# liruihui/Dis-PU

Measured on AMD Instinct MI355X. Metric: upsampled points/sec (256->1024, 4x), higher is better.
Workload: dtype f32; 1 GPU; BASELINE configs[1]: 32 patches x 256 points per GPU, generator forward 256->1024 (4x), fp32; patches_per_gpu=32, global_patches=32, weights=xavier-uniform seed 1234, zero bias, parallelism=patch-sharded x1

## Files before the change

dis-pu_amd/csrc/edge.hip:

```cpp
#include "common.h"
#include "knn_select.h"


namespace dispu {

typedef float f32x16 __attribute__((ext_vector_type(16)));

template <int CTRL>
__device__ __forceinline__ float edge_dpp(float identity, float v) {
    return __int_as_float(__builtin_amdgcn_update_dpp(__float_as_int(identity), __float_as_int(v), CTRL, 0xF, 0xF, false));
}
__device__ __forceinline__ float edge_row16_max(float v) {
    v = fmaxf(v, edge_dpp<0x121>(v, v));
    v = fmaxf(v, edge_dpp<0x122>(v, v));
    v = fmaxf(v, edge_dpp<0x124>(v, v));
    v = fmaxf(v, edge_dpp<0x128>(v, v));
    return v;
}

__device__ __forceinline__ void edge_fill_frag(float* frag, const float* __restrict__ W, int K, int tid, int nthreads) {
    const int nf4 = K * 24 / 4;
    for (int e = tid; e < nf4; e += nthreads) {
        const float4 v = *reinterpret_cast<const float4*>(W + e * 4);
        const int k = (e * 4) / 24, ch0 = (e * 4) - k * 24;
        const float vv[4] = {v.x, v.y, v.z, v.w};
#pragma unroll
        for (int u = 0; u < 4; ++u) {
            const int ch = ch0 + u, r = ch >> 1, hp = ch & 1;
            const int i = (r & 3) | (hp << 2) | ((r >> 2) << 3);
            frag[(k >> 1) * 64 + (k & 1) * 32 + i] = vv[u];
        }
    }
    for (int e = tid; e < K * 8; e += nthreads) {
        const int sh = e >> 3;
        frag[sh * 32 + 24 + (e & 7)] = 0.f;
    }
}

__device__ __forceinline__ void edge_scatter_f4(float* frag, int e, const float4 v) {
    const int k = (e * 4) / 24, ch0 = (e * 4) - k * 24;
    const float vv[4] = {v.x, v.y, v.z, v.w};
#pragma unroll
    for (int u = 0; u < 4; ++u) {
        const int ch = ch0 + u, r = ch >> 1, hp = ch & 1;
        const int i = (r & 3) | (hp << 2) | ((r >> 2) << 3);
        frag[(k >> 1) * 64 + (k & 1) * 32 + i] = vv[u];
    }
}

constexpr int EK_NP = 64 * 4 + 4;
constexpr int EK_SCRATCH = 128 + 4;
constexpr int EK_KLD = 20;
// ... 68 lines not shown
                        const float x = xr[k];
                        const float4 w = *reinterpret_cast<const float4*>(Wl + k * 24 + q * 4);
                        acc.x = __builtin_fmaf(x, w.x, acc.x); acc.y = __builtin_fmaf(x, w.y, acc.y);
                        acc.z = __builtin_fmaf(x, w.z, acc.z); acc.w = __builtin_fmaf(x, w.w, acc.w);
                    }
                    const float4 b = *reinterpret_cast<const float4*>(bl + q * 4);
                    acc.x = acc.x + b.x; acc.y = acc.y + b.y; acc.z = acc.z + b.z; acc.w = acc.w + b.w;
                    cv[u] = acc;
                    const int pl = p - (g_lo * 2 - cloud0);
                    if (e < ctotal && pl >= 0 && pl < (g_hi - g_lo) * 2)
                        *reinterpret_cast<float4*>(Lout + (size_t)(cloud0 + p) * ldl + q * 4) = acc;
                }
            }
        } else {
#pragma unroll
            for (int u = 0; u < CB; ++u) {
                const int e = min((int)threadIdx.x + u * NT, ctotal - 1);
                const int p = e / (C / 4), q = e - p * (C / 4);
                cv[u] = *reinterpret_cast<const float4*>(F + (size_t)(cloud0 + p) * ldf + q * 4);
            }
        }
#pragma unroll
        for (int u = 0; u < WB; ++u) {
            const int e = (int)threadIdx.x + u * NT;
            if (e < N0) edge_scatter_f4(f0, e, wv[u]);
            else if (e < N0 + N1) edge_scatter_f4(f1, e - N0, wv[u]);
            else if (e < N0 + N1 + N2) edge_scatter_f4(f2, e - N0 - N1, wv[u]);
        }
        for (int e = threadIdx.x; e < (K0 + K1 + K2) * 8; e += NT)
            frag[(e >> 3) * 32 + 24 + (e & 7)] = 0.f;
#pragma unroll
        for (int u = 0; u < CB; ++u) {
            const int e = (int)threadIdx.x + u * NT;
            const int p = e / (C / 4), q = e - p * (C / 4);
            if (e < ctotal) *reinterpret_cast<float4*>(fl + p * FLD + q * 4) = cv[u];
        }
        if (!layer0)
            for (int e = threadIdx.x + CB * NT; e < ctotal; e += NT) {
                const int p = e / (C / 4), q = e - p * (C / 4);
                *reinterpret_cast<float4*>(fl + p * FLD + q * 4) = *reinterpret_cast<const float4*>(F + (size_t)(cloud0 + p) * ldf + q * 4);
            }
    }
    __syncthreads();
#ifdef EDGE_STAMPS
    const unsigned long long e_ka = __builtin_readcyclecounter();
    unsigned long long e_kb = e_ka, e_kc = e_ka;
#endif
    const int lane = threadIdx.x & 63, wave = threadIdx.x >> 6;
    const int row = lane & 31, h = lane >> 5;
    float* pre = fl + n_per_cloud * FLD;
    float* norms = pre + per_wg * 2 * 24;
    uint32_t* dmat = reinterpret_cast<uint32_t*>(norms + ((n_per_cloud + 3) & ~3));
    uint64_t* kscr = reinterpret_cast<uint64_t*>(dmat + EK_MAXQ * EK_NP);
    int* nbr = reinterpret_cast<int*>(kscr + NWAVE * EK_SCRATCH);
    const int n = n_per_cloud, p_base = g_lo * 2 - cloud0, ngl = g_hi - g_lo, nq = ngl * 2;
    typedef float ek_f32x4 __attribute__((ext_vector_type(4)));
    ek_f32x4 d00 = {0.f, 0.f, 0.f, 0.f}, d01 = d00, d10 = d00, d11 = d00;
    const int i16 = lane & 15, q4 = lane >> 4;
    const int ntile = (n + 15) >> 4;
    if constexpr (KNN) {
        for (int p = threadIdx.x; p < n; p += 64 * NWAVE) {
            const float* fr = fl + p * FLD;
            float r = 0.f;
#pragma unroll
            for (int c4 = 0; c4 < C / 4; ++c4) {
                const float4 v = *reinterpret_cast<const float4*>(fr + c4 * 4);
                r = __builtin_fmaf(v.x, v.x, r); r = __builtin_fmaf(v.y, v.y, r);
                r = __builtin_fmaf(v.z, v.z, r); r = __builtin_fmaf(v.w, v.w, r);
            }
            norms[p] = r;
        }
        if (wave < ntile) {
            const float* q0row = fl + min(p_base + i16, n - 1) * FLD + q4;
            const float* q1row = fl + min(p_base + 16 + i16, n - 1) * FLD + q4;
            const float* c0p = fl + min(wave * 16 + i16, n - 1) * FLD + q4;
            const float* c1p = fl + min((wave + NWAVE) * 16 + i16, n - 1) * FLD + q4;
#pragma unroll
            for (int c4 = 0; c4 < C / 4; ++c4) {
                const float a0 = q0row[c4 * 4], a1 = q1row[c4 * 4], b0v = c0p[c4 * 4], b1v = c1p[c4 * 4];
                d00 = __builtin_amdgcn_mfma_f32_16x16x4f32(a0, b0v, d00, 0, 0, 0);
                d01 = __builtin_amdgcn_mfma_f32_16x16x4f32(a0, b1v, d01, 0, 0, 0);
                d10 = __builtin_amdgcn_mfma_f32_16x16x4f32(a1, b0v, d10, 0, 0, 0);
                d11 = __builtin_amdgcn_mfma_f32_16x16x4f32(a1, b1v, d11, 0, 0, 0);
            }
        }
    }
    if constexpr (PRE) {
        const int npts_wg = nq;
        const int tw = KNN ? NWAVE - 1 - wave : wave;
        for (int t = tw; t * 32 < npts_wg; t += NWAVE) {
            const int pl = min(t * 32 + row, npts_wg - 1);
            const float* fr = fl + (p_base + pl) * FLD;
            f32x16 acc;
#pragma unroll
            for (int r = 0; r < 16; ++r) acc[r] = 0.f;
#pragma unroll
            for (int sq = 0; sq < C / 4; ++sq) {
                const float4 a = *reinterpret_cast<const float4*>(fr + sq * 4);
                acc = __builtin_amdgcn_mfma_f32_32x32x2f32(f0[(2 * sq) * 64 + lane], h ? a.y : a.x, acc, 0, 0, 0);
                acc = __builtin_amdgcn_mfma_f32_32x32x2f32(f0[(2 * sq + 1) * 64 + lane], h ? a.w : a.z, acc, 0, 0, 0);
            }
            if (t * 32 + row < npts_wg) {
                float* pp = pre + ((t * 32 + row) * 2 + h) * 12;
#pragma unroll
                for (int q = 0; q < 3; ++q)
                    *reinterpret_cast<float4*>(pp + q * 4) = make_float4(acc[4 * q], acc[4 * q + 1], acc[4 * q + 2], acc[4 * q + 3]);
            }
        }
        __syncthreads();
    }
#ifdef EDGE_STAMPS
    e_kb = __builtin_readcyclecounter();
#endif
    if constexpr (KNN) {
        if (wave < ntile) {
            const int cand0 = wave * 16 + i16, cand1 = cand0 + NWAVE * 16;
            const float rp0 = norms[min(cand0, n - 1)], rp1 = norms[min(cand1, n - 1)];
#pragma unroll
            for (int r = 0; r < 4; ++r) {
                const float rq0 = norms[min(p_base + 4 * q4 + r, n - 1)], rq1 = norms[min(p_base + 16 + 4 * q4 + r, n - 1)];
                uint32_t* m0 = dmat + (4 * q4 + r) * EK_NP;
                uint32_t* m1 = m0 + 16 * EK_NP;
                if (cand0 < n) {
                    m0[cand0] = f32_to_ordered(((rq0 - 2.0f * d00[r]) + rp0) + 0.0f);
                    if (nq > 16) m1[cand0] = f32_to_ordered(((rq1 - 2.0f * d10[r]) + rp0) + 0.0f);
                }
                if (cand1 < n) {
                    m0[cand1] = f32_to_ordered(((rq0 - 2.0f * d01[r]) + rp1) + 0.0f);
                    if (nq > 16) m1[cand1] = f32_to_ordered(((rq1 - 2.0f * d11[r]) + rp1) + 0.0f);
                }
            }
        }
        __syncthreads();
#ifdef EDGE_STAMPS
        e_kc = __builtin_readcyclecounter();
#endif
    }
    auto knn_select = [&](int gl) {
        if constexpr (KNN) {
            const int qa = 2 * gl, qb = qa + 1;
            uint32_t oda[4], odb[4];
            int cp[4];
#pragma unroll
            for (int r = 0; r < 4; ++r) {
                const int p = lane + 64 * r;
                cp[r] = p;
                oda[r] = (p < n) ? dmat[qa * EK_NP + p] : 0xFFFFFFFFu;
                odb[r] = (p < n) ? dmat[qb * EK_NP + p] : 0xFFFFFFFFu;
            }
            uint64_t* buf = kscr + (size_t)wave * EK_SCRATCH;
            int* outa = nbr + qa * EK_KLD;
            int* outb = nbr + qb * EK_KLD;
            const auto w2f = [](uint32_t w) { return ordered_to_f32(w); };
            const bool done_a = prefilter_rank<4, true>(oda, cp, buf, lane, ksel, 0xFFFFFFFEu, outa, nullptr, w2f);
            const bool done_b = prefilter_rank<4, true>(odb, cp, buf, lane, ksel, 0xFFFFFFFEu, outb, nullptr, w2f);
            if (!(done_a && done_b)) {
                uint64_t ka[4], kb[4];
#pragma unroll
                for (int r = 0; r < 4; ++r) {
                    ka[r] = (cp[r] < n) ? (((uint64_t)oda[r] << 32) | (uint32_t)cp[r]) : KEY_MAX;
                    kb[r] = (cp[r] < n) ? (((uint64_t)odb[r] << 32) | (uint32_t)cp[r]) : KEY_MAX;
                }
                sort_keys<4>(ka);
                sort_keys<4>(kb);
                uint64_t resa, resb;
                select_k2<4>(ka, kb, lane, ksel, resa, resb);
                if (lane < ksel) {
                    if (!done_a) outa[lane] = (int)(uint32_t)resa;
                    if (!done_b) outb[lane] = (int)(uint32_t)resb;
                }
            }
            if (idx_out != nullptr && lane < ksel) {
                int* o = idx_out + (size_t)(cloud0 + p_base + qa) * ksel;
                o[lane] = outa[lane];
                o[ksel + lane] = outb[lane];
            }
        }
    };
    if constexpr (KNN) {
        for (int gl = wave; gl < ngl; gl += NWAVE) knn_select(gl);
    }
#ifdef EDGE_STAMPS
    const unsigned long long e_k1 = __builtin_readcyclecounter();
#endif

    const int ngroups = LDSF ? g_hi : (npoints + 1) / 2;
    const int s_nb = row & 15;
    float4 ra[LDSF ? 1 : C / 4], rb[LDSF ? 1 : C / 4];
    int jl_next = 0;
    auto fetch = [&](int grp) {
        int p = grp * 2 + (row >> 4);
        if (p >= npoints) p = npoints - 1;
        if constexpr (KNN) {
            jl_next = nbr[(p - g_lo * 2) * EK_KLD + ioff + s_nb];
        } else if constexpr (LDSF) {
            jl_next = idx[(size_t)p * ldi + ioff + s_nb];
        } else {
            const int j = (p / n_per_cloud) * n_per_cloud + idx[(size_t)p * ldi + ioff + s_nb];
#pragma unroll
            for (int q = 0; q < C / 4; ++q) {
                ra[q] = *reinterpret_cast<const float4*>(F + (size_t)p * ldf + q * 4);
                rb[q] = *reinterpret_cast<const float4*>(F + (size_t)j * ldf + q * 4);
            }
        }
    };
    const int grp0 = gfirst + wave, gstride = gstep0;
    if (grp0 < ngroups) fetch(grp0);
    constexpr int SKIP = PRE ? H : 0;
    constexpr int WD = 12, STOT = S0 + S1 + S2 - SKIP;
    static_assert(STOT % WD == 0, "fragment ring depth must divide the step count");
    const float* fragG = frag + SKIP * 64;
    float wq[WD];
#pragma unroll
    for (int i = 0; i < WD; ++i) wq[i] = fragG[i * 64 + lane];
#ifdef EDGE_STAMPS
    unsigned long long e_conv = 0, e_l0 = 0, e_l1 = 0, e_l2 = 0, e_epi = 0, e_n = 0;
#define ED_T(v) __builtin_amdgcn_sched_barrier(0); const unsigned long long v = __builtin_readcyclecounter(); __builtin_amdgcn_sched_barrier(0)
#else
#define ED_T(v)
#endif
    float tail_bias = 0.f;
    if constexpr (KNN) {
        if (Wp != nullptr) tail_bias = bp[min(wave >> 1, 2) * 16 + i16];
    }
    for (int grp = grp0; grp < ngroups; grp += gstride) {
        ED_T(t0);
        float fp[H], df[H];
        const float* fp_ = fl + (grp * 2 + (row >> 4) - cloud0) * FLD;
        const float* fj_ = fl + jl_next * FLD;
#pragma unroll
        for (int q = 0; q < C / 4; ++q) {
            const float4 a = LDSF ? *reinterpret_cast<const float4*>(fp_ + q * 4) : ra[q];
            const float4 b = LDSF ? *reinterpret_cast<const float4*>(fj_ + q * 4) : rb[q];
            const float a0 = h ? a.y : a.x, a1 = h ? a.w : a.z;
            const float b0v = h ? b.y : b.x, b1v = h ? b.w : b.z;
            fp[2 * q] = a0; fp[2 * q + 1] = a1;
            df[2 * q] = b0v - a0; df[2 * q + 1] = b1v - a1;
        }
        if (grp + gstride < ngroups) fetch(grp + gstride);
        f32x16 l0, l1, l2;
#pragma unroll
        for (int r = 0; r < 16; ++r) { l0[r] = 0.f; l1[r] = 0.f; l2[r] = 0.f; }
        if constexpr (PRE) {
            const float* pp = pre + (((grp - g_lo) * 2 + (row >> 4)) * 2 + h) * 12;
#pragma unroll
            for (int q = 0; q < 3; ++q) {
                const float4 v = *reinterpret_cast<const float4*>(pp + q * 4);
                l0[4 * q] = v.x; l0[4 * q + 1] = v.y; l0[4 * q + 2] = v.z; l0[4 * q + 3] = v.w;
            }
        }
        auto step = [&](int sg, float bv, f32x16& acc) {
            const float w = wq[sg % WD];
            wq[sg % WD] = fragG[((sg + WD) % STOT) * 64 + lane];
            acc = __builtin_amdgcn_mfma_f32_32x32x2f32(w, bv, acc, 0, 0, 0);
        };
        ED_T(t1);
#pragma unroll
        for (int s = SKIP; s < S0; ++s) {
            const float bv = (s < H) ? fp[s < H ? s : 0] : df[s < H ? 0 : s - H];
            step(s - SKIP, bv, l0);
        }
#pragma unroll
        for (int r = 0; r < 12; ++r) l0[r] = fmaxf(l0[r] + b0[2 * r + h], 0.f);
        ED_T(t2);
#pragma unroll
        for (int s = 0; s < S1; ++s) {
            const float bv = (s < 12) ? l0[s < 12 ? s : 0] : fp[s < 12 ? 0 : s - 12];
            step(S0 - SKIP + s, bv, l1);
        }
#pragma unroll
        for (int r = 0; r < 12; ++r) l1[r] = fmaxf(l1[r] + b1[2 * r + h], 0.f);
        ED_T(t3);
#pragma unroll
        for (int s = 0; s < S2; ++s) {
            const float bv = (s < 12) ? l1[s < 12 ? s : 0] : ((s < 24) ? l0[(s >= 12 && s < 24) ? s - 12 : 0] : fp[s >= 24 ? s - 24 : 0]);
            step(S0 + S1 - SKIP + s, bv, l2);
        }
// ... 1 lines not shown
        constexpr int OW = 3 * G + C;
        float* stg = stage + (KNN ? (grp - g_lo) : wave) * (2 * OWS);
        float* sp = stg + (row >> 4) * OWS;
        float k2 = 0.f, k1 = 0.f, k0 = 0.f;
#pragma unroll
        for (int r = 0; r < 12; ++r) {
            float m2 = l2[r] + b2[2 * r + h], m1 = l1[r], m0 = l0[r];
            asm("s_nop 1\n\t"
                "v_max_f32_dpp %0, %0, %0 row_ror:1 row_mask:0xf bank_mask:0xf\n\t"
                "v_max_f32_dpp %1, %1, %1 row_ror:1 row_mask:0xf bank_mask:0xf\n\t"
                "v_max_f32_dpp %2, %2, %2 row_ror:1 row_mask:0xf bank_mask:0xf\n\t"
                "v_max_f32_dpp %0, %0, %0 row_ror:2 row_mask:0xf bank_mask:0xf\n\t"
                "v_max_f32_dpp %1, %1, %1 row_ror:2 row_mask:0xf bank_mask:0xf\n\t"
                "v_max_f32_dpp %2, %2, %2 row_ror:2 row_mask:0xf bank_mask:0xf\n\t"
                "v_max_f32_dpp %0, %0, %0 row_ror:4 row_mask:0xf bank_mask:0xf\n\t"
                "v_max_f32_dpp %1, %1, %1 row_ror:4 row_mask:0xf bank_mask:0xf\n\t"
                "v_max_f32_dpp %2, %2, %2 row_ror:4 row_mask:0xf bank_mask:0xf\n\t"
                "v_max_f32_dpp %0, %0, %0 row_ror:8 row_mask:0xf bank_mask:0xf\n\t"
                "v_max_f32_dpp %1, %1, %1 row_ror:8 row_mask:0xf bank_mask:0xf\n\t"
                "v_max_f32_dpp %2, %2, %2 row_ror:8 row_mask:0xf bank_mask:0xf"
                : "+v"(m2), "+v"(m1), "+v"(m0));
            k2 = (s_nb == r) ? m2 : k2; k1 = (s_nb == r) ? m1 : k1; k0 = (s_nb == r) ? m0 : k0;
        }
        if (s_nb < 12) { sp[2 * s_nb + h] = k2; sp[G + 2 * s_nb + h] = k1; sp[2 * G + 2 * s_nb + h] = k0; }
        {
            float fa = 0.f, fb = 0.f;
#pragma unroll
            for (int t = 0; t < H; ++t) {
                if (t < 16) fa = (s_nb == t) ? fp[t] : fa;
                else fb = (s_nb == t - 16) ? fp[t] : fb;
            }
            if (s_nb < (H < 16 ? H : 16)) sp[3 * G + 2 * s_nb + h] = fa;
            if (H > 16 && s_nb < H - 16) sp[3 * G + 2 * (s_nb + 16) + h] = fb;
        }
        const int p_first = grp * 2;
        if (vec_store) {
            if (lane < 2 * (OW / 4)) {
                const int pt = lane / (OW / 4), q4 = lane - pt * (OW / 4);
                if (p_first + pt < npoints)
                    *reinterpret_cast<float4*>(Y + (size_t)(p_first + pt) * ldy + q4 * 4) = *reinterpret_cast<const float4*>(stg + pt * OWS + q4 * 4);
            }
        } else {
            for (int e = lane; e < 2 * OW; e += 64) {
                const int pt = e / OW, q = e - pt * OW;
                if (p_first + pt < npoints) Y[(size_t)(p_first + pt) * ldy + q] = stg[pt * OWS + q];
            }
        }
#ifdef EDGE_STAMPS
        { ED_T(t5); e_conv += t1 - t0; e_l0 += t2 - t1; e_l1 += t3 - t2; e_l2 += t4 - t3; e_epi += t5 - t4; ++e_n; }
#endif
    }
#ifdef EDGE_STAMPS
    const unsigned long long e_p0 = __builtin_readcyclecounter();
    unsigned long long e_p1 = e_p0, e_p2 = e_p0, e_p3 = e_p0;
#endif
    if constexpr (KNN) {
        if (Wp != nullptr) {
            constexpr int OW = 3 * G + C, NT = 64 * NWAVE;
            const int K = OW + k_old, xld = k_old + 4;
            float* wl = fl;
            float* xl = frag;
            __syncthreads();
#ifdef EDGE_STAMPS
            e_p1 = __builtin_readcyclecounter();
#endif
            const int wtot = K * 12, xq = k_old >> 2, xtot = nq * xq;
            constexpr int TB_W = 9, TB_X = 4;
            float4 wv[TB_W], xv[TB_X];
#pragma unroll
            for (int u = 0; u < TB_W; ++u) wv[u] = *reinterpret_cast<const float4*>(Wp + (size_t)min((int)threadIdx.x + u * NT, wtot - 1) * 4);
#pragma unroll
            for (int u = 0; u < TB_X; ++u) {
                const int e = min((int)threadIdx.x + u * NT, max(xtot - 1, 0));
                const int pl = xq ? e / xq : 0, c4 = e - pl * xq;
                xv[u] = xtot ? *reinterpret_cast<const float4*>(Y + (size_t)(g_lo * 2 + pl) * ldy + OW + c4 * 4) : make_float4(0.f, 0.f, 0.f, 0.f);
            }
#pragma unroll
            for (int u = 0; u < TB_W; ++u) {
                const int e = (int)threadIdx.x + u * NT;
                if (e < wtot) *reinterpret_cast<float4*>(wl + e * 4) = wv[u];
            }
#pragma unroll
            for (int u = 0; u < TB_X; ++u) {
                const int e = (int)threadIdx.x + u * NT;
                const int pl = xq ? e / xq : 0, c4 = e - pl * xq;
                if (e < xtot) *reinterpret_cast<float4*>(xl + pl * xld + c4 * 4) = xv[u];
            }
            for (int e = threadIdx.x + TB_W * NT; e < wtot; e += NT)
                *reinterpret_cast<float4*>(wl + e * 4) = *reinterpret_cast<const float4*>(Wp + (size_t)e * 4);
            for (int e = threadIdx.x + TB_X * NT; e < xtot; e += NT) {
                const int pl = e / xq, c4 = e - pl * xq;
                *reinterpret_cast<float4*>(xl + pl * xld + c4 * 4) = *reinterpret_cast<const float4*>(Y + (size_t)(g_lo * 2 + pl) * ldy + OW + c4 * 4);
            }
            __syncthreads();
#ifdef EDGE_STAMPS
            e_p2 = __builtin_readcyclecounter();
#endif
            const int pt = wave & 1, ct = wave >> 1;
            if (ct < 3 && pt * 16 < nq) {
                const int pl = min(pt * 16 + i16, nq - 1);
                const float* xn = stage + pl * OWS + q4;
                const float* xo = xl + pl * xld + q4;
                const float* wp = wl + q4 * 48 + ct * 16 + i16;
                ek_f32x4 acc = {0.f, 0.f, 0.f, 0.f};
                const int nround = K / 24;
                float av[6], bv[6], an[6], bn[6];
                auto rd_load = [&](int rd, float (&a)[6], float (&b)[6]) {
                    rd = min(rd, nround - 1);
                    const float* xa = (rd < OW / 24) ? xn + rd * 24 : xo + (rd - OW / 24) * 24;
                    const float* wb = wp + rd * 24 * 48;
#pragma unroll
                    for (int u = 0; u < 6; ++u) { a[u] = xa[u * 4]; b[u] = wb[u * 4 * 48]; }
                };
                rd_load(0, av, bv);
                for (int rd = 0; rd < nround; rd += 2) {
                    rd_load(rd + 1, an, bn);
#pragma unroll
                    for (int u = 0; u < 6; ++u) acc = __builtin_amdgcn_mfma_f32_16x16x4f32(av[u], bv[u], acc, 0, 0, 0);
                    if (rd + 1 < nround) {
                        rd_load(rd + 2, av, bv);
#pragma unroll
                        for (int u = 0; u < 6; ++u) acc = __builtin_amdgcn_mfma_f32_16x16x4f32(an[u], bn[u], acc, 0, 0, 0);
                    }
                }
#ifdef EDGE_STAMPS
                __builtin_amdgcn_sched_barrier(0); e_p3 = __builtin_readcyclecounter(); __builtin_amdgcn_sched_barrier(0);
#endif
                const float bb = tail_bias;
#pragma unroll
                for (int r = 0; r < 4; ++r) {
                    const int pr = pt * 16 + 4 * q4 + r;
                    if (pr < nq) Pout[(size_t)(g_lo * 2 + pr) * ldp + ct * 16 + i16] = fmaxf(acc[r] + bb, 0.f);
                }
            }
        }
    }
#ifdef EDGE_STAMPS
    if (blockIdx.x == 3 && blockIdx.y == 0 && lane == 0) {
        unsigned long long* st = reinterpret_cast<unsigned long long*>(Y + (size_t)npoints * ldy) + wave * 16;
        st[11] = e_p1 - e_p0; st[12] = e_p2 - e_p1; st[13] = __builtin_readcyclecounter() - e_p2; st[14] = e_p3 - e_p2;
        st[0] = e_conv; st[1] = e_l0; st[2] = e_l1; st[3] = e_l2; st[4] = e_epi; st[5] = e_n; st[6] = e_ka - e_k0; st[7] = e_kb - e_ka;
        st[8] = e_kc - e_kb; st[9] = e_k1 - e_kc; st[10] = __builtin_readcyclecounter() - e_k0;
    }
#endif
}

}

using namespace dispu;

DISPU_EXPORT int dispu_edge_dense_conv(int npoints, int n_per_cloud, int C, const float* F, long ldf, const int* idx, int ldi,
                                       int ioff, const float* W0, const float* b0, const float* W1, const float* b1,
                                       const float* W2, const float* b2, float* Y, long ldy, void* stream) {
    if (npoints < 0 || n_per_cloud <= 0 || !(C == 24 || C == 48) || (ldf & 3) || (((uintptr_t)F) & 15)) return (int)hipErrorInvalidValue;
    if (npoints == 0) return 0;
    hipStream_t s = (hipStream_t)stream;
    const size_t frag_bytes = (size_t)((C == 24 ? 84 : 132) * 64 + 16 * (72 + C)) * sizeof(float);
    const size_t feat_bytes = (size_t)n_per_cloud * (C + 4) * sizeof(float);
    if (npoints % n_per_cloud == 0 && n_per_cloud % 2 == 0 && frag_bytes + feat_bytes <= 160 * 1024) {
        const int clouds = npoints / n_per_cloud;
        int parts = (256 + clouds - 1) / clouds;
        const int gpc = n_per_cloud / 2;
        if (parts > (gpc + 7) / 8) parts = (gpc + 7) / 8;
        if (parts < 1) parts = 1;
        const int per = (gpc + parts - 1) / parts;
        const size_t pre_bytes = (size_t)per * 2 * 24 * sizeof(float);
        const bool pre = frag_bytes + feat_bytes + pre_bytes <= 160 * 1024;
        const size_t bytes = frag_bytes + feat_bytes + (pre ? pre_bytes : 0);
        static DevOnce attr;      
        if (attr.needed()) {
            DISPU_TRY(hipFuncSetAttribute(reinterpret_cast<const void*>(edge_dense_conv_mfma_kernel<24, true>),
                                          hipFuncAttributeMaxDynamicSharedMemorySize, 160 * 1024));
            DISPU_TRY(hipFuncSetAttribute(reinterpret_cast<const void*>(edge_dense_conv_mfma_kernel<48, true>),
                                          hipFuncAttributeMaxDynamicSharedMemorySize, 160 * 1024));
            DISPU_TRY(hipFuncSetAttribute(reinterpret_cast<const void*>(edge_dense_conv_mfma_kernel<24, true, true>),
                                          hipFuncAttributeMaxDynamicSharedMemorySize, 160 * 1024));
            DISPU_TRY(hipFuncSetAttribute(reinterpret_cast<const void*>(edge_dense_conv_mfma_kernel<48, true, true>),
                                          hipFuncAttributeMaxDynamicSharedMemorySize, 160 * 1024));
            attr.done();
        }
#define EDGE_LAUNCH(C_, PRE_) hipLaunchKernelGGL((edge_dense_conv_mfma_kernel<C_, true, PRE_>), dim3(clouds, parts), dim3(512), bytes, s, npoints, \
                                                 n_per_cloud, F, ldf, idx, ldi, ioff, W0, b0, W1, b1, W2, b2, Y, ldy, nullptr, 0, nullptr, nullptr, 0, nullptr, 0, nullptr, nullptr, nullptr, nullptr, 0)
        if (C == 24) { if (pre) EDGE_LAUNCH(24, true); else EDGE_LAUNCH(24, false); }
        else { if (pre) EDGE_LAUNCH(48, true); else EDGE_LAUNCH(48, false); }
#undef EDGE_LAUNCH
        return (int)hipGetLastError();
    }
    int g = (npoints + 7) / 8;
    if (g > 256) g = 256;
    if (C == 24)
        hipLaunchKernelGGL((edge_dense_conv_mfma_kernel<24, false>), dim3(g), dim3(256), frag_bytes, s, npoints, n_per_cloud, F, ldf, idx, ldi, ioff, W0, b0, W1, b1, W2, b2, Y, ldy, nullptr, 0, nullptr, nullptr, 0, nullptr, 0, nullptr, nullptr, nullptr, nullptr, 0);
    else
        hipLaunchKernelGGL((edge_dense_conv_mfma_kernel<48, false>), dim3(g), dim3(256), frag_bytes, s, npoints, n_per_cloud, F, ldf, idx, ldi, ioff, W0, b0, W1, b1, W2, b2, Y, ldy, nullptr, 0, nullptr, nullptr, 0, nullptr, 0, nullptr, nullptr, nullptr, nullptr, 0);
    return (int)hipGetLastError();
}

DISPU_EXPORT int dispu_linear(int batch, int M, int K, int N, const float* X, long ldx, long sx, const float* W, long ldw, long sw, int transb,
                              const float* bias, int act, float* Y, long ldy, long sy, const float* R1, long ldr1, long sr1, const float* R2,
                              long ldr2, long sr2, void* stream);

DISPU_EXPORT int dispu_stem_block(int npoints, int n_per_cloud, int C, const float* F, long ldf, int ksel, int ioff, const float* W0,
                                  const float* b0, const float* W1, const float* b1, const float* W2, const float* b2, float* Y, long ldy,
                                  int* idx_out, const float* Wp, const float* bp, int k_old, float* P, long ldp, const float* xyz,
                                  const float* Wl, const float* bl, float* Lout, long ldl, void* stream) {
    if (xyz != nullptr && (C != 24 || Wl == nullptr || bl == nullptr || Lout == nullptr || (ldl & 3) || (((uintptr_t)Lout) & 15) ||
                           (((uintptr_t)Wl) & 15) || (((uintptr_t)bl) & 15) || n_per_cloud * 6 > 8 * 512))
        return (int)hipErrorInvalidValue;
    if (xyz == nullptr && F == nullptr) return (int)hipErrorInvalidValue;
    if (Wp != nullptr && (bp == nullptr || P == nullptr || k_old < 0 || k_old % 24 != 0 || ldp < 48)) return (int)hipErrorInvalidValue;
    if (npoints < 0 || n_per_cloud <= 0 || !(C == 24 || C == 48) || (ldf & 3) || (((uintptr_t)F) & 15)) return (int)hipErrorInvalidValue;
    if (n_per_cloud > 256 || (n_per_cloud & 1) || npoints % n_per_cloud != 0 || ioff < 0 || ksel != ioff + 16 || ksel > EK_KLD ||
        ksel > n_per_cloud)
        return (int)hipErrorInvalidValue;
    if (npoints == 0) return 0;
    hipStream_t s = (hipStream_t)stream;
    const int clouds = npoints / n_per_cloud, gpc = n_per_cloud / 2;
    int parts = (256 + clouds - 1) / clouds;
    if (parts > (gpc + 7) / 8) parts = (gpc + 7) / 8;
    if (parts < (gpc + EK_MAXQ / 2 - 1) / (EK_MAXQ / 2)) parts = (gpc + EK_MAXQ / 2 - 1) / (EK_MAXQ / 2);
    const int per = (gpc + parts - 1) / parts;
    const float* Wp_fused = Wp;
    if (Wp != nullptr) {
        const long wcap = (long)n_per_cloud * (C + 4) + per * 48 + ((n_per_cloud + 3) & ~3) + EK_MAXQ * EK_NP, xcap = (C == 24 ? 84 : 132) * 64;
        if ((ldy & 3) || (((uintptr_t)Y) & 15) || (((uintptr_t)Wp) & 15)) return (int)hipErrorInvalidValue;
        if ((long)(72 + C + k_old) * 48 > wcap || (long)per * 2 * (k_old + 4) > xcap) Wp_fused = nullptr;
    }
    const size_t bytes = (size_t)((C == 24 ? 84 : 132) * 64 + EK_MAXQ * (72 + C + 4)) * sizeof(float) + (size_t)n_per_cloud * (C + 4) * sizeof(float) +
                         (size_t)per * 2 * 24 * sizeof(float) + (size_t)((n_per_cloud + 3) & ~3) * sizeof(float) +
                         (size_t)EK_MAXQ * EK_NP * sizeof(uint32_t) + (size_t)8 * EK_SCRATCH * sizeof(uint64_t) + (size_t)EK_MAXQ * EK_KLD * sizeof(int);
    static DevOnce attr;
    if (attr.needed()) {
        DISPU_TRY(hipFuncSetAttribute(reinterpret_cast<const void*>(edge_dense_conv_mfma_kernel<24, true, true, true>),
                                      hipFuncAttributeMaxDynamicSharedMemorySize, 160 * 1024));
        DISPU_TRY(hipFuncSetAttribute(reinterpret_cast<const void*>(edge_dense_conv_mfma_kernel<48, true, true, true>),
                                      hipFuncAttributeMaxDynamicSharedMemorySize, 160 * 1024));
        attr.done();
    }
    if (C == 24)
        hipLaunchKernelGGL((edge_dense_conv_mfma_kernel<24, true, true, true>), dim3(clouds, parts), dim3(512), bytes, s, npoints, n_per_cloud, F, ldf,
                           nullptr, 0, ioff, W0, b0, W1, b1, W2, b2, Y, ldy, idx_out, ksel, Wp_fused, bp, k_old, P, ldp, xyz, Wl, bl, Lout, ldl);
    else
        hipLaunchKernelGGL((edge_dense_conv_mfma_kernel<48, true, true, true>), dim3(clouds, parts), dim3(512), bytes, s, npoints, n_per_cloud, F, ldf,
                           nullptr, 0, ioff, W0, b0, W1, b1, W2, b2, Y, ldy, idx_out, ksel, Wp_fused, bp, k_old, P, ldp, xyz, Wl, bl, Lout, ldl);
    const int rc = (int)hipGetLastError();
    if (rc != 0 || Wp == Wp_fused) return rc;
    return dispu_linear(1, npoints, 72 + C + k_old, 48, Y, ldy, 0, Wp, 48, 0, 0, bp, 1, P, ldp, 0, nullptr, 0, 0, nullptr, 0, 0, stream);
}
```

dis-pu_amd/csrc/knn_select.h:

```cpp
#pragma once
#include "common.h"

namespace dispu {

constexpr uint64_t KEY_MAX = ~0ull;

__device__ __forceinline__ void cswap(uint64_t& a, uint64_t& b) {
    const bool c = a > b;
    const uint64_t lo = c ? b : a, hi = c ? a : b;
    a = lo; b = hi;
}

template <int R>
__device__ __forceinline__ void sort_keys(uint64_t (&a)[R]) {
#pragma unroll
    for (int p = 1; p < R; p <<= 1)
#pragma unroll
        for (int k = p; k >= 1; k >>= 1)
#pragma unroll
            for (int j = k % p; j <= R - 1 - k; j += 2 * k)
#pragma unroll
                for (int i = 0; i < k; ++i)
                    if (i + j + k < R && (i + j) / (2 * p) == (i + j + k) / (2 * p)) cswap(a[i + j], a[i + j + k]);
}
// ... 87 lines not shown
                                               unsigned long long* pf_stamps = nullptr) {
    constexpr int CAP = 128;
    PF_STAMP(0);
    uint32_t dmin = od[0];
#pragma unroll
    for (int r = 1; r < R; ++r) dmin = min(dmin, od[r]);
    uint32_t T = (uint32_t)__builtin_amdgcn_readlane((int)wave_bitonic_sort_u32(dmin, lane), k - 1);
    T = min(T, tmax);
    PF_STAMP(1);
    int cnt = 0;
#pragma unroll
    for (int r = 0; r < R; ++r) {
        const bool flag = od[r] <= T;
        const unsigned long long mk = __ballot(flag);
        const int pos = (int)__builtin_amdgcn_mbcnt_hi((unsigned)(mk >> 32), __builtin_amdgcn_mbcnt_lo((unsigned)mk, 0u));
        if (flag && (!GUARD || cnt + pos < CAP)) (buf + cnt)[pos] = ((uint64_t)od[r] << 32) | (uint32_t)cp[r];
        cnt += __popcll(mk);
    }
    PF_STAMP(2);
    if (cnt < k || cnt > CAP) return false;
    if (lane < 4) buf[cnt + lane] = KEY_MAX;
    const uint64_t m0 = (lane < cnt) ? buf[lane] : KEY_MAX;
    if (cnt <= 64) {
        int r0 = 0;
        for (int j = 0; j < cnt; j += 4) {
            const uint64_t a0 = buf[j], a1 = buf[j + 1], a2 = buf[j + 2], a3 = buf[j + 3];
            r0 += (int)(a0 < m0) + (int)(a1 < m0) + (int)(a2 < m0) + (int)(a3 < m0);
        }
        if (r0 < k) {
            idx_out[r0] = (int)(uint32_t)m0;
            if (dist_out) dist_out[r0] = word_to_float((uint32_t)(m0 >> 32));
        }
    } else {
        const uint64_t m1 = (lane + 64 < cnt) ? buf[lane + 64] : KEY_MAX;
        int r0 = 0, r1 = 0;
        for (int j = 0; j < cnt; j += 4) {
            const uint64_t a0 = buf[j], a1 = buf[j + 1], a2 = buf[j + 2], a3 = buf[j + 3];
            r0 += (int)(a0 < m0) + (int)(a1 < m0) + (int)(a2 < m0) + (int)(a3 < m0);
            r1 += (int)(a0 < m1) + (int)(a1 < m1) + (int)(a2 < m1) + (int)(a3 < m1);
        }
        if (r0 < k) {
            idx_out[r0] = (int)(uint32_t)m0;
            if (dist_out) dist_out[r0] = word_to_float((uint32_t)(m0 >> 32));
        }
        if (r1 < k) {
            idx_out[r1] = (int)(uint32_t)m1;
            if (dist_out) dist_out[r1] = word_to_float((uint32_t)(m1 >> 32));
        }
    }
    PF_STAMP(3);
    return true;
}

template <int R>
__device__ __forceinline__ void select_k2(const uint64_t (&ka)[R], const uint64_t (&kb)[R], int lane, int k, uint64_t& ra, uint64_t& rb) {
    static_assert(R <= 4, "register-resident selection is written for up to four keys per lane");
    uint32_t hda = (uint32_t)(ka[0] >> 32), hia = (uint32_t)ka[0], hdb = (uint32_t)(kb[0] >> 32), hib = (uint32_t)kb[0];
    int hpa = 0, hpb = 0;
    ra = 0; rb = 0;
    auto nth = [&](const uint64_t (&key)[R], int hp) -> uint64_t {
        uint64_t v = KEY_MAX;
#pragma unroll
        for (int i = R - 1; i >= 1; --i) v = (hp == i) ? key[i] : v;
        return v;
    };
    for (int t = 0; t < k; ++t) {
        const uint32_t mda = wave_min_u32(hda), mdb = wave_min_u32(hdb);
        unsigned long long ma = __ballot(hda == mda), mb = __ballot(hdb == mdb);
        if (__popcll(ma) != 1) {
            const uint32_t mi = wave_min_u32(hda == mda ? hia : 0xFFFFFFFFu);
            ma = __ballot(hda == mda && hia == mi);
        }
        if (__popcll(mb) != 1) {
            const uint32_t mi = wave_min_u32(hdb == mdb ? hib : 0xFFFFFFFFu);
            mb = __ballot(hdb == mdb && hib == mi);
        }
        const int wa = __builtin_ctzll(ma), wb = __builtin_ctzll(mb);
        const uint32_t wia = (uint32_t)__builtin_amdgcn_readlane((int)hia, wa), wib = (uint32_t)__builtin_amdgcn_readlane((int)hib, wb);
        if (lane == t) { ra = ((uint64_t)mda << 32) | wia; rb = ((uint64_t)mdb << 32) | wib; }
        if (lane == wa) { ++hpa; const uint64_t nk = nth(ka, hpa); hda = (uint32_t)(nk >> 32); hia = (uint32_t)nk; }
        if (lane == wb) { ++hpb; const uint64_t nk = nth(kb, hpb); hdb = (uint32_t)(nk >> 32); hib = (uint32_t)nk; }
    }
}

}
```

Measured before the change: 36.11 million points/s.

## Pair kNN prefilter for two queries and widen tail projection MFMA tiles

Replaces the two separate per-query prefilter_rank calls with a joint prefilter_rank2. It sorts both queries' per-lane minima together in one wave-wide DPP/swizzle bitonic network, derives thresholds, and compacts candidates into separate per-query scratch buffers, which doubles the scratch allocation. The fused tail projection is rewritten with inline-asm ds_read and MFMA sequences, and some waves now compute two 16-column output tiles at once. The global-to-LDS loads are also hoisted ahead of the barrier. This trades more LDS and hand-scheduled asm (fixed s_nop/waitcnt hazards) for fewer serialized wave reductions and better MFMA overlap.

```diff
diff --git a/dis-pu_amd/csrc/edge.hip b/dis-pu_amd/csrc/edge.hip
--- a/dis-pu_amd/csrc/edge.hip
+++ b/dis-pu_amd/csrc/edge.hip
@@ -1,3 +1,4 @@
+#include <type_traits>
 #include "common.h"
 #include "knn_select.h"
 
@@ -172,7 +173,7 @@
     float* norms = pre + per_wg * 2 * 24;
     uint32_t* dmat = reinterpret_cast<uint32_t*>(norms + ((n_per_cloud + 3) & ~3));
     uint64_t* kscr = reinterpret_cast<uint64_t*>(dmat + EK_MAXQ * EK_NP);
-    int* nbr = reinterpret_cast<int*>(kscr + NWAVE * EK_SCRATCH);
+    int* nbr = reinterpret_cast<int*>(kscr + NWAVE * 2 * EK_SCRATCH);
     const int n = n_per_cloud, p_base = g_lo * 2 - cloud0, ngl = g_hi - g_lo, nq = ngl * 2;
     typedef float ek_f32x4 __attribute__((ext_vector_type(4)));
     ek_f32x4 d00 = {0.f, 0.f, 0.f, 0.f}, d01 = d00, d10 = d00, d11 = d00;
@@ -268,12 +269,11 @@
                 oda[r] = (p < n) ? dmat[qa * EK_NP + p] : 0xFFFFFFFFu;
                 odb[r] = (p < n) ? dmat[qb * EK_NP + p] : 0xFFFFFFFFu;
             }
-            uint64_t* buf = kscr + (size_t)wave * EK_SCRATCH;
+            uint64_t* buf = kscr + (size_t)wave * (2 * EK_SCRATCH);
             int* outa = nbr + qa * EK_KLD;
             int* outb = nbr + qb * EK_KLD;
-            const auto w2f = [](uint32_t w) { return ordered_to_f32(w); };
-            const bool done_a = prefilter_rank<4, true>(oda, cp, buf, lane, ksel, 0xFFFFFFFEu, outa, nullptr, w2f);
-            const bool done_b = prefilter_rank<4, true>(odb, cp, buf, lane, ksel, 0xFFFFFFFEu, outb, nullptr, w2f);
+            bool done_a, done_b;
+            prefilter_rank2<4>(oda, odb, cp, buf, buf + EK_SCRATCH, lane, ksel, 0xFFFFFFFEu, outa, outb, done_a, done_b);
             if (!(done_a && done_b)) {
                 uint64_t ka[4], kb[4];
 #pragma unroll
@@ -339,10 +339,6 @@
 #else
 #define ED_T(v)
 #endif
-    float tail_bias = 0.f;
-    if constexpr (KNN) {
-        if (Wp != nullptr) tail_bias = bp[min(wave >> 1, 2) * 16 + i16];
-    }
     for (int grp = grp0; grp < ngroups; grp += gstride) {
         ED_T(t0);
         float fp[H], df[H];
@@ -450,7 +446,7 @@
     }
 #ifdef EDGE_STAMPS
     const unsigned long long e_p0 = __builtin_readcyclecounter();
-    unsigned long long e_p1 = e_p0, e_p2 = e_p0, e_p3 = e_p0;
+    unsigned long long e_p1 = e_p0, e_p2 = e_p0, e_p3 = 0;
 #endif
     if constexpr (KNN) {
         if (Wp != nullptr) {
@@ -458,31 +454,36 @@
             const int K = OW + k_old, xld = k_old + 4;
             float* wl = fl;
             float* xl = frag;
-            __syncthreads();
-#ifdef EDGE_STAMPS
-            e_p1 = __builtin_readcyclecounter();
-#endif
             const int wtot = K * 12, xq = k_old >> 2, xtot = nq * xq;
             constexpr int TB_W = 9, TB_X = 4;
-            float4 wv[TB_W], xv[TB_X];
-#pragma unroll
-            for (int u = 0; u < TB_W; ++u) wv[u] = *reinterpret_cast<const float4*>(Wp + (size_t)min((int)threadIdx.x + u * NT, wtot - 1) * 4);
+            ek_f32x4 wv[TB_W], xv[TB_X];
+#pragma unroll
+            for (int u = 0; u < TB_W; ++u) wv[u] = *reinterpret_cast<const ek_f32x4*>(Wp + (size_t)min((int)threadIdx.x + u * NT, wtot - 1) * 4);
 #pragma unroll
             for (int u = 0; u < TB_X; ++u) {
                 const int e = min((int)threadIdx.x + u * NT, max(xtot - 1, 0));
                 const int pl = xq ? e / xq : 0, c4 = e - pl * xq;
-                xv[u] = xtot ? *reinterpret_cast<const float4*>(Y + (size_t)(g_lo * 2 + pl) * ldy + OW + c4 * 4) : make_float4(0.f, 0.f, 0.f, 0.f);
-            }
+                xv[u] = ek_f32x4{0.f, 0.f, 0.f, 0.f};
+                if (xtot) xv[u] = *reinterpret_cast<const ek_f32x4*>(Y + (size_t)(g_lo * 2 + pl) * ldy + OW + c4 * 4);
+            }
+            const bool t_pts2 = nq > 16;
+            const int t_pt = t_pts2 ? (wave & 1) : 0, t_ct = min(t_pts2 ? (wave >> 1) * 2 : wave, 2);
+            const bool t_own = wave < (t_pts2 ? 4 : 3), t_two = t_pts2 && wave < 2;
+            const float bias_a = bp[t_ct * 16 + i16], bias_b = bp[min(t_ct + 1, 2) * 16 + i16];
+            __syncthreads();
+#ifdef EDGE_STAMPS
+            e_p1 = __builtin_readcyclecounter();
+#endif
 #pragma unroll
             for (int u = 0; u < TB_W; ++u) {
                 const int e = (int)threadIdx.x + u * NT;
-                if (e < wtot) *reinterpret_cast<float4*>(wl + e * 4) = wv[u];
+                if (e < wtot) *reinterpret_cast<ek_f32x4*>(wl + e * 4) = wv[u];
             }
 #pragma unroll
             for (int u = 0; u < TB_X; ++u) {
                 const int e = (int)threadIdx.x + u * NT;
                 const int pl = xq ? e / xq : 0, c4 = e - pl * xq;
-                if (e < xtot) *reinterpret_cast<float4*>(xl + pl * xld + c4 * 4) = xv[u];
+                if (e < xtot) *reinterpret_cast<ek_f32x4*>(xl + pl * xld + c4 * 4) = xv[u];
             }
             for (int e = threadIdx.x + TB_W * NT; e < wtot; e += NT)
                 *reinterpret_cast<float4*>(wl + e * 4) = *reinterpret_cast<const float4*>(Wp + (size_t)e * 4);
@@ -494,49 +495,100 @@
 #ifdef EDGE_STAMPS
             e_p2 = __builtin_readcyclecounter();
 #endif
-            const int pt = wave & 1, ct = wave >> 1;
-            if (ct < 3 && pt * 16 < nq) {
-                const int pl = min(pt * 16 + i16, nq - 1);
+            if (t_own) {
+                const int pl = min(t_pt * 16 + i16, nq - 1);
                 const float* xn = stage + pl * OWS + q4;
                 const float* xo = xl + pl * xld + q4;
-                const float* wp = wl + q4 * 48 + ct * 16 + i16;
-                ek_f32x4 acc = {0.f, 0.f, 0.f, 0.f};
+                const float* wp = wl + q4 * 48 + t_ct * 16 + i16;
                 const int nround = K / 24;
-                float av[6], bv[6], an[6], bn[6];
-                auto rd_load = [&](int rd, float (&a)[6], float (&b)[6]) {
-                    rd = min(rd, nround - 1);
-                    const float* xa = (rd < OW / 24) ? xn + rd * 24 : xo + (rd - OW / 24) * 24;
-                    const float* wb = wp + rd * 24 * 48;
-#pragma unroll
-                    for (int u = 0; u < 6; ++u) { a[u] = xa[u * 4]; b[u] = wb[u * 4 * 48]; }
+                auto tiles = [&](auto two_c) __attribute__((always_inline)) {
+                    constexpr bool TWO = decltype(two_c)::value;
+                    constexpr int NB = TWO ? 6 : 1;
+                    ek_f32x4 acc = {0.f, 0.f, 0.f, 0.f}, acd = acc;
+                    float av[6], bv[6], dv[NB], an[6], bn[6], dn[NB];
+                    auto rd_load = [&](int rd, float (&a)[6], float (&b)[6], float (&d)[NB]) __attribute__((always_inline)) {
+                        rd = min(rd, nround - 1);
+                        const float* xa = (rd < OW / 24) ? xn + rd * 24 : xo + (rd - OW / 24) * 24;
+                        const float* wb = wp + rd * 24 * 48;
+#pragma unroll
+                        for (int u = 0; u < 6; ++u) {
+                            a[u] = xa[u * 4]; b[u] = wb[u * 4 * 48];
+                            if constexpr (TWO) d[u] = wb[u * 4 * 48 + 16];
+                        }
+                    };
+                    typedef const __attribute__((address_space(3))) float* lds_cptr;
+                    rd_load(0, av, bv, dv);
+                    asm volatile("" : "+v"(av[0]), "+v"(av[1]), "+v"(av[2]), "+v"(av[3]), "+v"(av[4]), "+v"(av[5]),
+                                      "+v"(bv[0]), "+v"(bv[1]), "+v"(bv[2]), "+v"(bv[3]), "+v"(bv[4]), "+v"(bv[5]));
+                    if constexpr (TWO)
+                        asm volatile("" : "+v"(dv[0]), "+v"(dv[1 % NB]), "+v"(dv[2 % NB]), "+v"(dv[3 % NB]), "+v"(dv[4 % NB]), "+v"(dv[5 % NB]));
+                    for (int rd = 0; rd < nround; ++rd) {
+                        const int rn = min(rd + 1, nround - 1);
+                        const uint32_t xa = (uint32_t)(uintptr_t)(lds_cptr)((rn < OW / 24) ? xn + rn * 24 : xo + (rn - OW / 24) * 24);
+                        const uint32_t wb = (uint32_t)(uintptr_t)(lds_cptr)(wp + rn * 24 * 48);
+                        asm volatile("ds_read_b32 %0, %12\n\tds_read_b32 %1, %12 offset:16\n\tds_read_b32 %2, %12 offset:32\n\t"
+                                     "ds_read_b32 %3, %12 offset:48\n\tds_read_b32 %4, %12 offset:64\n\tds_read_b32 %5, %12 offset:80\n\t"
+                                     "ds_read_b32 %6, %13\n\tds_read_b32 %7, %13 offset:768\n\tds_read_b32 %8, %13 offset:1536\n\t"
+                                     "ds_read_b32 %9, %13 offset:2304\n\tds_read_b32 %10, %13 offset:3072\n\tds_read_b32 %11, %13 offset:3840"
+                                     : "=&v"(an[0]), "=&v"(an[1]), "=&v"(an[2]), "=&v"(an[3]), "=&v"(an[4]), "=&v"(an[5]),
+                                       "=&v"(bn[0]), "=&v"(bn[1]), "=&v"(bn[2]), "=&v"(bn[3]), "=&v"(bn[4]), "=&v"(bn[5])
+                                     : "v"(xa), "v"(wb) : "memory");
+                        if constexpr (TWO) {
+                            asm volatile("ds_read_b32 %0, %6 offset:64\n\tds_read_b32 %1, %6 offset:832\n\tds_read_b32 %2, %6 offset:1600\n\t"
+                                         "ds_read_b32 %3, %6 offset:2368\n\tds_read_b32 %4, %6 offset:3136\n\tds_read_b32 %5, %6 offset:3904"
+                                         : "=&v"(dn[0]), "=&v"(dn[1 % NB]), "=&v"(dn[2 % NB]), "=&v"(dn[3 % NB]), "=&v"(dn[4 % NB]), "=&v"(dn[5 % NB])
+                                         : "v"(wb) : "memory");
+                            asm volatile("v_mfma_f32_16x16x4_f32 %0, %2, %8, %0\n\tv_mfma_f32_16x16x4_f32 %1, %2, %14, %1\n\t"
+                                         "v_mfma_f32_16x16x4_f32 %0, %3, %9, %0\n\tv_mfma_f32_16x16x4_f32 %1, %3, %15, %1\n\t"
+                                         "v_mfma_f32_16x16x4_f32 %0, %4, %10, %0\n\tv_mfma_f32_16x16x4_f32 %1, %4, %16, %1\n\t"
+                                         "v_mfma_f32_16x16x4_f32 %0, %5, %11, %0\n\tv_mfma_f32_16x16x4_f32 %1, %5, %17, %1\n\t"
+                                         "v_mfma_f32_16x16x4_f32 %0, %6, %12, %0\n\tv_mfma_f32_16x16x4_f32 %1, %6, %18, %1\n\t"
+                                         "v_mfma_f32_16x16x4_f32 %0, %7, %13, %0\n\tv_mfma_f32_16x16x4_f32 %1, %7, %19, %1"
+                                         : "+v"(acc), "+v"(acd)
+                                         : "v"(av[0]), "v"(av[1]), "v"(av[2]), "v"(av[3]), "v"(av[4]), "v"(av[5]),
+                                           "v"(bv[0]), "v"(bv[1]), "v"(bv[2]), "v"(bv[3]), "v"(bv[4]), "v"(bv[5]),
+                                           "v"(dv[0]), "v"(dv[1 % NB]), "v"(dv[2 % NB]), "v"(dv[3 % NB]), "v"(dv[4 % NB]), "v"(dv[5 % NB]));
+                            asm volatile("s_waitcnt lgkmcnt(0)"
+                                         : "+v"(dn[0]), "+v"(dn[1 % NB]), "+v"(dn[2 % NB]), "+v"(dn[3 % NB]), "+v"(dn[4 % NB]), "+v"(dn[5 % NB]));
+                        } else {
+                            asm volatile("v_mfma_f32_16x16x4_f32 %0, %1, %7, %0\n\tv_mfma_f32_16x16x4_f32 %0, %2, %8, %0\n\t"
+                                         "v_mfma_f32_16x16x4_f32 %0, %3, %9, %0\n\tv_mfma_f32_16x16x4_f32 %0, %4, %10, %0\n\t"
+                                         "v_mfma_f32_16x16x4_f32 %0, %5, %11, %0\n\tv_mfma_f32_16x16x4_f32 %0, %6, %12, %0"
+                                         : "+v"(acc)
+                                         : "v"(av[0]), "v"(av[1]), "v"(av[2]), "v"(av[3]), "v"(av[4]), "v"(av[5]),
+                                           "v"(bv[0]), "v"(bv[1]), "v"(bv[2]), "v"(bv[3]), "v"(bv[4]), "v"(bv[5]));
+                        }
+                        asm volatile("s_waitcnt lgkmcnt(0)"
+                                     : "+v"(an[0]), "+v"(an[1]), "+v"(an[2]), "+v"(an[3]), "+v"(an[4]), "+v"(an[5]),
+                                       "+v"(bn[0]), "+v"(bn[1]), "+v"(bn[2]), "+v"(bn[3]), "+v"(bn[4]), "+v"(bn[5]));
+#pragma unroll
+                        for (int u = 0; u < 6; ++u) { av[u] = an[u]; bv[u] = bn[u]; }
+#pragma unroll
+                        for (int u = 0; u < NB; ++u) dv[u] = dn[u];
+                    }
+                    asm volatile("s_nop 15\n\ts_nop 3" : "+v"(acc), "+v"(acd));
+#ifdef EDGE_STAMPS
+                    __builtin_amdgcn_sched_barrier(0); e_p3 = __builtin_readcyclecounter(); __builtin_amdgcn_sched_barrier(0);
+#endif
+#pragma unroll
+                    for (int r = 0; r < 4; ++r) {
+                        const int pr = t_pt * 16 + 4 * q4 + r;
+                        if (pr < nq) {
+                            float* po = Pout + (size_t)(g_lo * 2 + pr) * ldp + t_ct * 16 + i16;
+                            po[0] = fmaxf(acc[r] + bias_a, 0.f);
+                            if constexpr (TWO) po[16] = fmaxf(acd[r] + bias_b, 0.f);
+                        }
+                    }
                 };
-                rd_load(0, av, bv);
-                for (int rd = 0; rd < nround; rd += 2) {
-                    rd_load(rd + 1, an, bn);
-#pragma unroll
-                    for (int u = 0; u < 6; ++u) acc = __builtin_amdgcn_mfma_f32_16x16x4f32(av[u], bv[u], acc, 0, 0, 0);
-                    if (rd + 1 < nround) {
-                        rd_load(rd + 2, av, bv);
-#pragma unroll
-                        for (int u = 0; u < 6; ++u) acc = __builtin_amdgcn_mfma_f32_16x16x4f32(an[u], bn[u], acc, 0, 0, 0);
-                    }
-                }
-#ifdef EDGE_STAMPS
-                __builtin_amdgcn_sched_barrier(0); e_p3 = __builtin_readcyclecounter(); __builtin_amdgcn_sched_barrier(0);
-#endif
-                const float bb = tail_bias;
-#pragma unroll
-                for (int r = 0; r < 4; ++r) {
-                    const int pr = pt * 16 + 4 * q4 + r;
-                    if (pr < nq) Pout[(size_t)(g_lo * 2 + pr) * ldp + ct * 16 + i16] = fmaxf(acc[r] + bb, 0.f);
-                }
+                if (t_two) tiles(std::true_type{}); else tiles(std::false_type{});
             }
         }
     }
 #ifdef EDGE_STAMPS
     if (blockIdx.x == 3 && blockIdx.y == 0 && lane == 0) {
         unsigned long long* st = reinterpret_cast<unsigned long long*>(Y + (size_t)npoints * ldy) + wave * 16;
-        st[11] = e_p1 - e_p0; st[12] = e_p2 - e_p1; st[13] = __builtin_readcyclecounter() - e_p2; st[14] = e_p3 - e_p2;
+        st[11] = e_p1 - e_p0; st[12] = e_p2 - e_p1; st[13] = __builtin_readcyclecounter() - e_p2; st[14] = e_p3 ? e_p3 - e_p2 : 0;
+        st[15] = e_p0 - e_k0;
         st[0] = e_conv; st[1] = e_l0; st[2] = e_l1; st[3] = e_l2; st[4] = e_epi; st[5] = e_n; st[6] = e_ka - e_k0; st[7] = e_kb - e_ka;
         st[8] = e_kc - e_kb; st[9] = e_k1 - e_kc; st[10] = __builtin_readcyclecounter() - e_k0;
     }
@@ -625,7 +677,7 @@
     }
     const size_t bytes = (size_t)((C == 24 ? 84 : 132) * 64 + EK_MAXQ * (72 + C + 4)) * sizeof(float) + (size_t)n_per_cloud * (C + 4) * sizeof(float) +
                          (size_t)per * 2 * 24 * sizeof(float) + (size_t)((n_per_cloud + 3) & ~3) * sizeof(float) +
-                         (size_t)EK_MAXQ * EK_NP * sizeof(uint32_t) + (size_t)8 * EK_SCRATCH * sizeof(uint64_t) + (size_t)EK_MAXQ * EK_KLD * sizeof(int);
+                         (size_t)EK_MAXQ * EK_NP * sizeof(uint32_t) + (size_t)8 * 2 * EK_SCRATCH * sizeof(uint64_t) + (size_t)EK_MAXQ * EK_KLD * sizeof(int);
     static DevOnce attr;
     if (attr.needed()) {
         DISPU_TRY(hipFuncSetAttribute(reinterpret_cast<const void*>(edge_dense_conv_mfma_kernel<24, true, true, true>),
diff --git a/dis-pu_amd/csrc/knn_select.h b/dis-pu_amd/csrc/knn_select.h
--- a/dis-pu_amd/csrc/knn_select.h
+++ b/dis-pu_amd/csrc/knn_select.h
@@ -163,6 +163,121 @@
     return true;
 }
 
+#define DISPU_SORT2_BANK(a, b, ctl_lo, ctl_hi, bm_lo, bm_hi)                                                      \
+    {                                                                                                              \
+        uint32_t ta_, tb_;                                                                                         \
+        asm("s_nop 1\n\tv_min_u32_dpp %0, %2, %2 " ctl_lo " row_mask:0xf bank_mask:" bm_lo                         \
+            "\n\tv_min_u32_dpp %1, %3, %3 " ctl_lo " row_mask:0xf bank_mask:" bm_lo                                 \
+            "\n\tv_max_u32_dpp %0, %2, %2 " ctl_hi " row_mask:0xf bank_mask:" bm_hi                                 \
+            "\n\tv_max_u32_dpp %1, %3, %3 " ctl_hi " row_mask:0xf bank_mask:" bm_hi                                 \
+            : "=&v"(ta_), "=&v"(tb_) : "v"(a), "v"(b));                                                            \
+        a = ta_; b = tb_;                                                                                          \
+    }
+#define DISPU_SORT2_QUAD(a, b, perm, lower)                                                                       \
+    {                                                                                                              \
+        uint32_t la_, ha_, lb_, hb_;                                                                               \
+        asm("s_nop 1\n\tv_min_u32_dpp %0, %4, %4 quad_perm:" perm " row_mask:0xf bank_mask:0xf"                    \
+            "\n\tv_min_u32_dpp %2, %5, %5 quad_perm:" perm " row_mask:0xf bank_mask:0xf"                            \
+            "\n\tv_max_u32_dpp %1, %4, %4 quad_perm:" perm " row_mask:0xf bank_mask:0xf"                            \
+            "\n\tv_max_u32_dpp %3, %5, %5 quad_perm:" perm " row_mask:0xf bank_mask:0xf"                            \
+            : "=&v"(la_), "=&v"(ha_), "=&v"(lb_), "=&v"(hb_) : "v"(a), "v"(b));                                    \
+        a = (lower) ? la_ : ha_; b = (lower) ? lb_ : hb_;                                                          \
+    }
+#define DISPU_SORT2_X8(a, b) DISPU_SORT2_BANK(a, b, "row_ror:8", "row_ror:8", "0x3", "0xc")
+#define DISPU_SORT2_X4(a, b) DISPU_SORT2_BANK(a, b, "row_shl:4", "row_shr:4", "0x5", "0xa")
+#define DISPU_SORT2_X2(a, b) DISPU_SORT2_QUAD(a, b, "[2,3,0,1]", e2)
+#define DISPU_SORT2_X1(a, b) DISPU_SORT2_QUAD(a, b, "[1,0,3,2]", e1)
+__device__ __forceinline__ void wave_bitonic_sort2_u32(uint32_t& a, uint32_t& b, int lane) {
+    const bool e1 = (lane & 1) == 0, e2 = (lane & 2) == 0, e16 = (lane & 16) == 0, e32 = lane < 32;
+    DISPU_SORT2_X1(a, b);
+    DISPU_SORT2_QUAD(a, b, "[3,2,1,0]", e2); DISPU_SORT2_X1(a, b);
+    DISPU_SORT2_BANK(a, b, "row_half_mirror", "row_half_mirror", "0x5", "0xa"); DISPU_SORT2_X2(a, b); DISPU_SORT2_X1(a, b);
+    DISPU_SORT2_BANK(a, b, "row_mirror", "row_mirror", "0x3", "0xc"); DISPU_SORT2_X4(a, b); DISPU_SORT2_X2(a, b); DISPU_SORT2_X1(a, b);
+    {
+        const uint32_t oa = (uint32_t)__builtin_amdgcn_ds_swizzle((int)a, 0x7C1F), ob = (uint32_t)__builtin_amdgcn_ds_swizzle((int)b, 0x7C1F);
+        a = e16 ? min(a, oa) : max(a, oa);
+        b = e16 ? min(b, ob) : max(b, ob);
+    }
+    DISPU_SORT2_X8(a, b); DISPU_SORT2_X4(a, b); DISPU_SORT2_X2(a, b); DISPU_SORT2_X1(a, b);
+    {
+        uint32_t oa = (uint32_t)__builtin_amdgcn_ds_bpermute((63 - lane) * 4, (int)a), ob = (uint32_t)__builtin_amdgcn_ds_bpermute((63 - lane) * 4, (int)b);
+        a = e32 ? min(a, oa) : max(a, oa);
+        b = e32 ? min(b, ob) : max(b, ob);
+        oa = (uint32_t)__builtin_amdgcn_ds_swizzle((int)a, 0x401F);
+        ob = (uint32_t)__builtin_amdgcn_ds_swizzle((int)b, 0x401F);
+        a = e16 ? min(a, oa) : max(a, oa);
+        b = e16 ? min(b, ob) : max(b, ob);
+    }
+    DISPU_SORT2_X8(a, b); DISPU_SORT2_X4(a, b); DISPU_SORT2_X2(a, b); DISPU_SORT2_X1(a, b);
+}
+
+__device__ __forceinline__ void prefilter_rank_tail(uint64_t* buf, int cnt, int lane, int k, int* __restrict__ idx_out) {
+    if (lane < 4) buf[cnt + lane] = KEY_MAX;
+    const uint64_t m0 = (lane < cnt) ? buf[lane] : KEY_MAX;
+    const uint64_t m1 = (lane + 64 < cnt) ? buf[lane + 64] : KEY_MAX;
+    int r0 = 0, r1 = 0;
+    for (int j = 0; j < cnt; j += 4) {
+        const uint64_t a0 = buf[j], a1 = buf[j + 1], a2 = buf[j + 2], a3 = buf[j + 3];
+        r0 += (int)(a0 < m0) + (int)(a1 < m0) + (int)(a2 < m0) + (int)(a3 < m0);
+        r1 += (int)(a0 < m1) + (int)(a1 < m1) + (int)(a2 < m1) + (int)(a3 < m1);
+    }
+    if (r0 < k) idx_out[r0] = (int)(uint32_t)m0;
+    if (r1 < k) idx_out[r1] = (int)(uint32_t)m1;
+}
+
+template <int R>
+__device__ __forceinline__ void prefilter_rank2(const uint32_t (&oda)[R], const uint32_t (&odb)[R], const int (&cp)[R], uint64_t* bufa,
+                                                uint64_t* bufb, int lane, int k, uint32_t tmax, int* __restrict__ outa,
+                                                int* __restrict__ outb, bool& done_a, bool& done_b) {
+    constexpr int CAP = 128;
+    uint32_t mina = oda[0], minb = odb[0];
+#pragma unroll
+    for (int r = 1; r < R; ++r) { mina = min(mina, oda[r]); minb = min(minb, odb[r]); }
+    wave_bitonic_sort2_u32(mina, minb, lane);
+    const uint32_t Ta = min((uint32_t)__builtin_amdgcn_readlane((int)mina, k - 1), tmax);
+    const uint32_t Tb = min((uint32_t)__builtin_amdgcn_readlane((int)minb, k - 1), tmax);
+    int cnta = 0, cntb = 0;
+#pragma unroll
+    for (int r = 0; r < R; ++r) {
+        const bool fa = oda[r] <= Ta, fb = odb[r] <= Tb;
+        const unsigned long long ma = __ballot(fa), mb = __ballot(fb);
+        const int pa = (int)__builtin_amdgcn_mbcnt_hi((unsigned)(ma >> 32), __builtin_amdgcn_mbcnt_lo((unsigned)ma, 0u));
+        const int pb = (int)__builtin_amdgcn_mbcnt_hi((unsigned)(mb >> 32), __builtin_amdgcn_mbcnt_lo((unsigned)mb, 0u));
+        if (fa && cnta + pa < CAP) (bufa + cnta)[pa] = ((uint64_t)oda[r] << 32) | (uint32_t)cp[r];
+        if (fb && cntb + pb < CAP) (bufb + cntb)[pb] = ((uint64_t)odb[r] << 32) | (uint32_t)cp[r];
+        cnta += __popcll(ma);
+        cntb += __popcll(mb);
+    }
+    done_a = !(cnta < k || cnta > CAP);
+    done_b = !(cntb < k || cntb > CAP);
+    if (done_a && done_b && cnta <= 64 && cntb <= 64) {
+        if (lane < 4) { bufa[cnta + lane] = KEY_MAX; bufb[cntb + lane] = KEY_MAX; }
+        const uint64_t m0a = (lane < cnta) ? bufa[lane] : KEY_MAX, m0b = (lane < cntb) ? bufb[lane] : KEY_MAX;
+        int ra = 0, rb = 0;
+        const int cmin = min(cnta, cntb);
+        int j = 0;
+        for (; j < cmin; j += 4) {
+            const uint64_t a0 = bufa[j], a1 = bufa[j + 1], a2 = bufa[j + 2], a3 = bufa[j + 3];
+            const uint64_t b0 = bufb[j], b1 = bufb[j + 1], b2 = bufb[j + 2], b3 = bufb[j + 3];
+            ra += (int)(a0 < m0a) + (int)(a1 < m0a) + (int)(a2 < m0a) + (int)(a3 < m0a);
+            rb += (int)(b0 < m0b) + (int)(b1 < m0b) + (int)(b2 < m0b) + (int)(b3 < m0b);
+        }
+        for (int ja = j; ja < cnta; ja += 4) {
+            const uint64_t a0 = bufa[ja], a1 = bufa[ja + 1], a2 = bufa[ja + 2], a3 = bufa[ja + 3];
+            ra += (int)(a0 < m0a) + (int)(a1 < m0a) + (int)(a2 < m0a) + (int)(a3 < m0a);
+        }
+        for (int jb = j; jb < cntb; jb += 4) {
+            const uint64_t b0 = bufb[jb], b1 = bufb[jb + 1], b2 = bufb[jb + 2], b3 = bufb[jb + 3];
+            rb += (int)(b0 < m0b) + (int)(b1 < m0b) + (int)(b2 < m0b) + (int)(b3 < m0b);
+        }
+        if (ra < k) outa[ra] = (int)(uint32_t)m0a;
+        if (rb < k) outb[rb] = (int)(uint32_t)m0b;
+    } else {
+        if (done_a) prefilter_rank_tail(bufa, cnta, lane, k, outa);
+        if (done_b) prefilter_rank_tail(bufb, cntb, lane, k, outb);
+    }
+}
+
 template <int R>
 __device__ __forceinline__ void select_k2(const uint64_t (&ka)[R], const uint64_t (&kb)[R], int lane, int k, uint64_t& ra, uint64_t& rb) {
     static_assert(R <= 4, "register-resident selection is written for up to four keys per lane");
```

Result: no change. 36.24 million points/s, median of 6 (+0.3%).
